# SamShue/EKF_SLAM

Hardware: AMD Instinct MI355X
Metric: EKF update-steps/sec at N landmarks; HBM GB/s on (I−KH)P vs roofline (higher is better)
Workload: dtype f64

## Files before the change

ekf_slam_amd/csrc/downdate.h:

```cpp
#pragma once

template <typename TS, int T, int kSlab>
__global__ __launch_bounds__(kBlock) void k_downdate(const TS *__restrict__ tiles, TS *__restrict__ dst,
                                                     const int2 *__restrict__ work, int64_t nwork,
                                                     const double *__restrict__ Kp, const double *__restrict__ Gp,
                                                     int64_t pair_stride, int pstart, int pcap, int npairs, TileMap tm) {
    using V2 = typename Vec2<TS>::type;
    constexpr int kPairsPerRow = T / 2;
    constexpr int kRowsPerPass = kBlock / kPairsPerRow;
    constexpr int kSlabsPerTile = T / kSlab;
    constexpr int kPasses = (kSlab + kRowsPerPass - 1) / kRowsPerPass;
    constexpr bool kExact = kRowsPerPass * kPasses == kSlab;
    static_assert(kPasses <= 8, "slab too tall for the register tile");
    const int tid = threadIdx.x;
    const int cp = tid % kPairsPerRow;
    const int r0 = tid / kPairsPerRow;
    const int64_t nitems = nwork * kSlabsPerTile;
    for (int64_t it0 = blockIdx.x; it0 < nitems; it0 += gridDim.x) {
        const int64_t it = tm.reverse ? nitems - 1 - it0 : it0;
        const int64_t w = it / kSlabsPerTile;
        const int slab = (int)(it - w * kSlabsPerTile);
        const int2 ij = work[w];
        const int64_t toff = tm.tile_offset(ij.x, ij.y) + (int64_t)slab * kSlab * T;
        const TS *__restrict__ tp = tiles + toff;
        TS *__restrict__ td = dst + toff;
        double2 v[kPasses];
#pragma unroll
        for (int p = 0; p < kPasses; ++p) {
            const int r = r0 + p * kRowsPerPass;
            if (kExact || r < kSlab) {
                const V2 t = *reinterpret_cast<const V2 *>(tp + r * T + 2 * cp);
                v[p] = make_double2((double)t.x, (double)t.y);
            }
        }
        const int64_t gcol = (int64_t)ij.y * T + 2 * cp;
        const int64_t krow = (int64_t)ij.x * T + slab * kSlab;
        for (int i = 0; i < npairs; ++i) {
            const int64_t so = (int64_t)ring_slot(pstart, i, pcap) * pair_stride;
            const double2 *__restrict__ g2 = reinterpret_cast<const double2 *>(Gp + so) + gcol;
            const double2 *__restrict__ k2 = reinterpret_cast<const double2 *>(Kp + so) + krow;
            const double2 ga = g2[0], gb = g2[1];
#pragma unroll
            for (int p = 0; p < kPasses; ++p) {
                const int r = r0 + p * kRowsPerPass;
                if (kExact || r < kSlab) {
                    const double2 k = k2[r];
                    v[p].x = rank2_apply(v[p].x, k, ga);
                    v[p].y = rank2_apply(v[p].y, k, gb);
                }
            }
        }
#pragma unroll
        for (int p = 0; p < kPasses; ++p) {
            const int r = r0 + p * kRowsPerPass;
            if (kExact || r < kSlab) {
                V2 o;
                o.x = (TS)v[p].x; o.y = (TS)v[p].y;
                *reinterpret_cast<V2 *>(td + r * T + 2 * cp) = o;
            }
        }
    }
}

template <typename TS> struct Lane16;
template <> struct Lane16<double> { using type = double2; static constexpr int kCols = 2; };
template <> struct Lane16<float>  { using type = float4;  static constexpr int kCols = 4; };
__device__ __forceinline__ void lane16_unpack(const double2 &t, double *v) { v[0] = t.x; v[1] = t.y; }
__device__ __forceinline__ void lane16_unpack(const float4 &t, double *v) { v[0] = t.x; v[1] = t.y; v[2] = t.z; v[3] = t.w; }
__device__ __forceinline__ void lane16_pack(const double *v, double2 &t) { t.x = v[0]; t.y = v[1]; }
__device__ __forceinline__ void lane16_pack(const double *v, float4 &t) {
    t.x = (float)v[0]; t.y = (float)v[1]; t.z = (float)v[2]; t.w = (float)v[3];
}
__device__ __forceinline__ double lane16_get(const double2 &t, int q) { return q == 0 ? t.x : t.y; }
__device__ __forceinline__ double lane16_get(const float4 &t, int q) { return (double)(q == 0 ? t.x : q == 1 ? t.y : q == 2 ? t.z : t.w); }

__device__ __attribute__((noinline)) void extract_next_row(double *__restrict__ send, int jm, int Ij, int tI, int tJ, int r, int c0, int ncols,
                                                           int T, int world, int rank, double v0, double v1, double v2, double v3) {
    const uint32_t wd = (uint32_t)world;
    const int k0 = (int)(((uint32_t)rank + wd - (uint32_t)Ij % wd) % wd);
    const bool rowtile = tI == Ij, coltile = tJ == Ij, diag = rowtile && coltile;
    for (int q = 0; q < ncols; ++q) {
        const int cc = c0 + q;
        const double val = q == 0 ? v0 : q == 1 ? v1 : q == 2 ? v2 : v3;
        if (rowtile && (r == jm || r == jm + 1)) {
            const int a = r - jm;
            if (!diag || cc <= jm) {
                const int64_t e = (int64_t)((tJ - k0) / world) * T + cc;
                send[2 * e + a] = val;
            }
            if (diag && a == 1 && (cc == jm || cc == jm + 1)) {
                const int64_t e = (int64_t)((Ij - k0) / world) * T + jm + 1;
                send[2 * e + (cc - jm)] = val;
            }
        }
        if (coltile && (cc == jm || cc == jm + 1) && (tI > Ij || r > jm + 1)) {
            const int64_t e = (int64_t)((tI - k0) / world) * T + r;
            send[2 * e + (cc - jm)] = val;
        }
    }
}

struct NoNextRow {};
template <bool kNext> struct NextRowParam { using type = NoNextRow; };
template <> struct NextRowParam<true> { using type = NextRow; };

template <typename TS, int T, int kSlab, bool kXcd, bool kNext = false>
__global__ __launch_bounds__(kBlock) void k_downdate_w(const TS *__restrict__ tiles, TS *__restrict__ dst,
                                                       const int2 *__restrict__ work, int64_t nwork,
                                                       const double *__restrict__ Kp, const double *__restrict__ Gp,
                                                       int64_t pair_stride, int pstart, int pcap, int npairs, TileMap tm,
                                                       typename NextRowParam<kNext>::type nx) {
    using VL = typename Lane16<TS>::type;
    constexpr int kCols = Lane16<TS>::kCols;
    constexpr int kLanesPerRow = T / kCols;
    constexpr int kRowsPerInstr = 64 / kLanesPerRow;
    constexpr int kRowsPerWave = kSlab / 4;
    constexpr int kPasses = kRowsPerWave / kRowsPerInstr;
    constexpr int kSlabsPerTile = T / kSlab;
    static_assert(kLanesPerRow == 64 || kLanesPerRow == 32, "tile edge / storage type combination not supported");
    static_assert(kPasses >= 1 && kPasses <= 8 && kPasses * kRowsPerInstr * 4 == kSlab, "bad slab");
    const int lane = threadIdx.x & 63;
    const int wave = __builtin_amdgcn_readfirstlane(threadIdx.x >> 6);
    const int sub = lane / kLanesPerRow;
    const int cl = lane % kLanesPerRow;
    const int64_t nitems = (kXcd ? 8 : 1) * nwork * kSlabsPerTile;
    const int64_t nv = nwork * kSlabsPerTile;
    for (int64_t it = blockIdx.x; it < nitems; it += gridDim.x) {
        const int64_t vf = kXcd ? (it >> 3) : it;
        const int64_t vi = tm.reverse ? nv - 1 - vf : vf;
        const int64_t w = vi / kSlabsPerTile;
        const int slab = (int)(vi - w * kSlabsPerTile);
        const int2 ij = work[kXcd ? (it & 7) * nwork + w : w];
        if (kXcd && ij.x < 0) continue;
        const int row0 = slab * kSlab + wave * kRowsPerWave;
        const int64_t toff = tm.tile_offset(ij.x, ij.y) + (int64_t)(row0 + sub) * T + kCols * cl;
        const TS *__restrict__ tp = tiles + toff;
        TS *__restrict__ td = dst + toff;
        double v[kPasses][kCols];
#pragma unroll
        for (int p = 0; p < kPasses; ++p) {
            const VL t = *reinterpret_cast<const VL *>(tp + (int64_t)p * kRowsPerInstr * T);
            lane16_unpack(t, v[p]);
        }
        const int64_t gcol = (int64_t)ij.y * T + kCols * cl;
        const int64_t krow = (int64_t)ij.x * T + row0;
        for (int i = 0; i < npairs; ++i) {
            const int64_t so = (int64_t)ring_slot(pstart, i, pcap) * pair_stride;
            const double2 *__restrict__ g2 = reinterpret_cast<const double2 *>(Gp + so) + gcol;
            const double2 *__restrict__ k2 = reinterpret_cast<const double2 *>(Kp + so) + krow;
            double2 g[kCols];
#pragma unroll
            for (int q = 0; q < kCols; ++q) g[q] = g2[q];
#pragma unroll
            for (int p = 0; p < kPasses; ++p) {
                double2 k = k2[p * kRowsPerInstr];
                if (kRowsPerInstr == 2) { const double2 k1 = k2[p * 2 + 1]; if (sub) k = k1; }
#pragma unroll
                for (int q = 0; q < kCols; ++q) v[p][q] = rank2_apply(v[p][q], k, g[q]);
            }
        }
        VL stored[kPasses];
#pragma unroll
        for (int p = 0; p < kPasses; ++p) {
            lane16_pack(v[p], stored[p]);
            *reinterpret_cast<VL *>(td + (int64_t)p * kRowsPerInstr * T) = stored[p];
        }
        if constexpr (kNext) {
            const int Ij = (int)(nx.j >> tm.shift);
            if (__builtin_expect(ij.x == Ij || ij.y == Ij, 0)) {
#pragma unroll
                for (int p = 0; p < kPasses; ++p) {
                    double vv[4] = { 0.0, 0.0, 0.0, 0.0 };
#pragma unroll
                    for (int q = 0; q < kCols; ++q) vv[q] = lane16_get(stored[p], q);
                    extract_next_row(nx.send, (int)(nx.j & (T - 1)), Ij, ij.x, ij.y, row0 + sub + p * kRowsPerInstr, kCols * cl, kCols, T,
                                     tm.world, tm.rank, vv[0], vv[1], vv[2], vv[3]);
                }
            }
        }
    }
}
```

ekf_slam_amd/csrc/flush64_mfma.h:

```cpp
#pragma once

typedef double d4_t __attribute__((ext_vector_type(4)));

template <typename TS, int T, int kChunk, int kCols = 128, int kWpe = (kChunk <= 4 ? 4 : 3), int kWaves = 4, int kAbl = 0>
__global__ __launch_bounds__(64 * kWaves) __attribute__((amdgpu_waves_per_eu(kWpe, kWpe)))
void k_flush_mfma(const TS *__restrict__ tiles, TS *__restrict__ dst, const int2 *__restrict__ work, int64_t nwork,
                  const double *__restrict__ Kp, const double *__restrict__ Gp, int64_t pair_stride, int pstart, int pcap,
                  int npairs, TileMap tm) {
    constexpr int kBlock = 64 * kWaves;
    constexpr int kRows = 16 * kWaves, kKPad = kRows + 16;
    constexpr int kE = 16 / (int)sizeof(TS);
    constexpr int kBP = kCols / (16 * kE);
    constexpr int kColParts = T / kCols, kSubsPerTile = (T / kRows) * kColParts;
    static_assert((kBP * kE == 8 || kBP * kE == 4) && T % kCols == 0 && T % kRows == 0, "a wavefront owns 16 rows x 128 (64) columns = 8 (4) MFMA blocks");
    static_assert(kChunk % 2 == 0 && (kChunk * kCols) % kBlock == 0 && (kChunk * kRows) % kBlock == 0, "bad chunk");
    __shared__ __attribute__((aligned(16))) double Gs[2 * kChunk][kCols];
    __shared__ double Ks[2 * kChunk][kKPad];
    const int tid = threadIdx.x;
    const int lane = tid & 63;
    const int wave = __builtin_amdgcn_readfirstlane(tid >> 6);
    const int lr = lane >> 4, lc = lane & 15;
    const int64_t nitems = 8 * nwork * kSubsPerTile;
    for (int64_t it = blockIdx.x; it < nitems; it += gridDim.x) {
        const int64_t vi = tm.reverse ? nwork * kSubsPerTile - 1 - (it >> 3) : (it >> 3);
        const int64_t w = vi / kSubsPerTile;
        const int sub = (int)(vi - w * kSubsPerTile);
        const int2 ij = work[(it & 7) * nwork + w];
        if (ij.x < 0) continue;
        const int slab = sub / kColParts, cpart = sub - slab * kColParts;
        const int row0 = slab * kRows + wave * 16;
        const int64_t toff = tm.tile_offset(ij.x, ij.y) + (int64_t)(row0 + lr) * T + cpart * kCols + kE * lc;
        const TS *__restrict__ tp = tiles + toff;
        TS *__restrict__ td = dst + toff;
        d4_t acc[kBP][kE];
#pragma unroll
        for (int bp = 0; bp < kBP; ++bp)
#pragma unroll
            for (int r = 0; r < 4; ++r)
#pragma unroll
                for (int e = 0; e < kE; ++e)
                    acc[bp][e][r] = (double)__builtin_nontemporal_load(tp + (int64_t)(4 * r) * T + 16 * kE * bp + e);
        const int64_t gcol0 = (int64_t)ij.y * T + cpart * kCols;
        const int64_t krow0 = (int64_t)ij.x * T + slab * kRows;
        constexpr int kPerG = kChunk * kCols / kBlock, kPerK = kChunk * kRows / kBlock;
        double2 tg[kPerG], tk[kPerK];
        auto fetch = [&](int c0, int cn) {
#pragma unroll
            for (int q = 0; q < kPerG; ++q) {
                const int e = tid + q * kBlock, col = e & (kCols - 1);
                const int i = (e / kCols) < cn ? (e / kCols) : cn - 1;
                tg[q] = reinterpret_cast<const double2 *>(Gp + (int64_t)ring_slot(pstart, c0 + i, pcap) * pair_stride)[gcol0 + col];
            }
#pragma unroll
            for (int q = 0; q < kPerK; ++q) {
                const int e = tid + q * kBlock, row = e & (kRows - 1);
                const int i = (e / kRows) < cn ? (e / kRows) : cn - 1;
                tk[q] = reinterpret_cast<const double2 *>(Kp + (int64_t)ring_slot(pstart, c0 + i, pcap) * pair_stride)[krow0 + row];
            }
        };
        if constexpr (kAbl < 2) fetch(0, npairs < kChunk ? npairs : kChunk);
        for (int c0 = 0; kAbl < 2 && c0 < npairs; c0 += kChunk) {
            const int cn = npairs - c0 < kChunk ? npairs - c0 : kChunk;
            __syncthreads();
#pragma unroll
            for (int q = 0; q < kPerG; ++q) {
                const int e = tid + q * kBlock, i = e / kCols, col = e & (kCols - 1);
                if (i < cn) { Gs[2 * i][col] = tg[q].x; Gs[2 * i + 1][col] = tg[q].y; }
                else if (i == cn) { Gs[2 * i][col] = 0.0; Gs[2 * i + 1][col] = 0.0; }
            }
#pragma unroll
            for (int q = 0; q < kPerK; ++q) {
                const int e = tid + q * kBlock, i = e / kRows, row = e & (kRows - 1);
                if (i < cn) { Ks[2 * i][row] = -tk[q].x; Ks[2 * i + 1][row] = -tk[q].y; }
                else if (i == cn) { Ks[2 * i][row] = -0.0; Ks[2 * i + 1][row] = -0.0; }
            }
            __syncthreads();
            if (c0 + kChunk < npairs) fetch(c0 + kChunk, npairs - c0 - kChunk < kChunk ? npairs - c0 - kChunk : kChunk);
            const int ksteps = kAbl ? 0 : (cn + 1) >> 1;
#pragma unroll 2
            for (int ks = 0; ks < ksteps; ++ks) {
                const double a = Ks[4 * ks + lr][wave * 16 + lc];
                double2 b[kBP][kE / 2];
// ... 27 lines not shown
```

ekf_slam_amd/csrc/host/handle.h:

```cpp
#pragma once
#include "../../../include/ekfslam.h"
#include <hip/hip_runtime.h>
#include <dlfcn.h>
#include <cstdio>
#include <cstdlib>
#include <algorithm>
#include <cmath>
#include <cstring>
#include <new>
#include <string>
#include <vector>

#include "../device_math.h"
#include "../flush32_pipe.h"
#include "../kernels.h"
#include "../layout.h"

struct KernelTimer {
    bool enabled = false;
    std::vector<hipEvent_t> ev;
    size_t used = 0;
};

struct ekf_handle {
    ekf_config cfg;
    int64_t N = 0;
    int64_t cap = 0;
    int32_t T = 64;
    int32_t storage = 0;
    int32_t cur = 0;
    DevState st;
    hipStream_t own_stream = nullptr, stream = nullptr;
    double *h_small = nullptr;
    double *d_digest = nullptr;
    bool have_pp = false;
    PredictArgs pp;
    std::vector<double> s_host;
    mutable std::vector<std::pair<double, int64_t>> s_sorted, s_tail;
    mutable bool s_sorted_ok = false;
    static constexpr size_t kSortedTail = 2048;
    hipEvent_t throttle_ev[2] = { nullptr, nullptr };
    bool throttle_set[2] = { false, false };
    int throttle_k = 0, since_mark = 0;
    int32_t batch = 1;
    int32_t npend = 0;
    int32_t pstart = 0;
    bool async_flush = false;
    void *tilebuf[2] = { nullptr, nullptr };
    int32_t base = 0;
    int32_t nfrozen = 0;
    bool inflight = false;
    int64_t inflight_N = 0;
    bool appended_inflight = false;
    const int64_t *inflight_dn = nullptr;
    int flush_cus = 0;
    hipStream_t flush_stream = nullptr;
    hipEvent_t ev_pairs = nullptr, ev_flushed = nullptr, ev_rows = nullptr;
    PassAux aux = { nullptr, 0, nullptr, 0, 0, nullptr, nullptr };
    int grid_cap = 0;
    char dd_kernel[64] = "";
    int32_t dd_pairs = 0;
    struct WorkSet {
        int2 *work = nullptr;
        int64_t nwork = 0;
        int2 *xcd = nullptr;
        int64_t xcd_len = 0;
        int4 *segs = nullptr;
        int64_t nsegs = 0, cols = 0;
        int64_t rows = -1;
    };
    WorkSet ws[2];
    int32_t ws_cur = 0;
    int32_t ws_pass = -1;
    bool ws_unordered = false;
    int64_t work_cap = 0, segs_cap = 0;
    char *wl_stage = nullptr;
    size_t wl_stage_bytes = 0;
    hipEvent_t ev_wl = nullptr;
    bool wl_busy = false;
    AssocDecision *d_partial = nullptr, *d_decision = nullptr, *h_decision = nullptr;
    AssocDecision *h_decision_dev = nullptr;
    int *d_ticket = nullptr;
    double *d_pos_cost = nullptr, *d_sig_cost = nullptr;
    int32_t assoc_seq = 0;
    static constexpr int kSpecRing = 64;
    AssocHostPartial *h_parts = nullptr, *h_parts_dev = nullptr;
    int64_t parts_stride = 0;
    bool assoc_poll = true;
    struct Spec { int32_t seq, is_new, nblk; int64_t idx, idx_N; };
    std::vector<Spec> spec;
    static constexpr int kLoopRing = 256;
    AssocHostPartial *d_lparts = nullptr;
    int64_t lparts_stride = 0;
    int32_t loop_set = 0;
    AssocHostPartial *h_lrec = nullptr, *h_lrec_dev = nullptr;
    struct LoopSpec { int32_t seq, is_new; int64_t idx; };
    std::vector<LoopSpec> lspec;
    uint64_t lrec_head = 0, lrec_tail = 0;
    static constexpr int kNRing = 1024;
    int64_t *d_nring = nullptr;
    uint64_t nrow = 0;
    static constexpr int kTabSets = 64, kTabCap = 512;
    double *h_loctab = nullptr, *h_loctab_dev = nullptr;
    int32_t *d_abort = nullptr;
    int32_t scan_id = 0;
    int64_t lookup_fail_hits = -1;
    uint64_t tab_until[kTabSets] = {};
    bool tab_used[kTabSets] = {};
    int tab_next = 0;
    bool sharded = false;
    double *own_send = nullptr, *own_recv = nullptr, *send = nullptr, *recv = nullptr;
    int64_t slab_cap = 0;
    int64_t xchg_cap = 0;
    int64_t slab = 0;
    bool pending = false;
    bool assoc_costs = false;
    int pending_kind = 0;
// ... 162 lines not shown
```

ekf_slam_amd/csrc/host/passes.h:

```cpp
#pragma once
namespace {
int32_t refresh_work(ekf_handle *h) {
    const int64_t nt = ekf_tiles_for(2 * n_hi(h), h->T);
    if (nt == h->ws[h->ws_cur].rows) return EKF_OK;
    const int32_t to = h->ws_pass == h->ws_cur ? h->ws_cur ^ 1 : h->ws_cur;
    ekf_handle::WorkSet &ws = h->ws[to];
    const size_t b_work = (size_t)h->work_cap * sizeof(int2), b_xcd = 8 * b_work, b_segs = (size_t)h->segs_cap * sizeof(int4);
    if (!h->wl_stage) h->wl_stage_bytes = b_work + b_xcd + b_segs;
    int32_t rc = stage_alloc(h, &h->wl_stage, h->wl_stage_bytes, &h->ev_wl);
    if (!rc) rc = stage_wait(h, h->ev_wl, h->wl_busy);
    if (rc) return rc;
    int2 *w = reinterpret_cast<int2 *>(h->wl_stage);
    int2 *flat = reinterpret_cast<int2 *>(h->wl_stage + b_work);
    int4 *segs = reinterpret_cast<int4 *>(h->wl_stage + b_work + b_xcd);
    size_t nw = 0;
    REQUIRE(h, h->st.tm.slots_for_rows(nt) <= h->work_cap, EKF_ERR_STATE, "work list overflow");
    for (int64_t I = 0; I < nt; ++I)
        for (int64_t J = 0; J <= I; ++J)
            if (h->st.tm.mine(I, J)) w[nw++] = make_int2((int)I, (int)J);
    if (nw) HIPCHK(h, hipMemcpyAsync(ws.work, w, nw * sizeof(int2), hipMemcpyHostToDevice, h->stream));
    ws.nwork = (int64_t)nw;
    ws.rows = nt;

    static const int S = std::max(1, ekf_tune_int("EKF_SUPERTILE", 8));
    struct Super { int64_t si, sj; std::vector<int2> tiles; };
    std::vector<Super> supers;
    const int64_t ns = (nt + S - 1) / S;
    for (int64_t si = 0; si < ns; ++si)
        for (int64_t sj = 0; sj <= si; ++sj) {
            Super sp; sp.si = si; sp.sj = sj;
            for (int64_t I = si * S; I < nt && I < (si + 1) * S; ++I)
                for (int64_t J = sj * S; J <= I && J < (sj + 1) * S; ++J)
                    if (h->st.tm.mine(I, J)) sp.tiles.push_back(make_int2((int)I, (int)J));
            if (!sp.tiles.empty()) supers.push_back(std::move(sp));
        }
    static const int order = ekf_tune_int("EKF_XCD_ORDER", 1);
    std::vector<int2> stream[8];
    if (order == 0) {
        std::stable_sort(supers.begin(), supers.end(), [](const Super &a, const Super &b) { return a.tiles.size() > b.tiles.size(); });
        for (const Super &sp : supers) {
            int best = 0;
            for (int x = 1; x < 8; ++x) if (stream[x].size() < stream[best].size()) best = x;
            stream[best].insert(stream[best].end(), sp.tiles.begin(), sp.tiles.end());
        }
    } else {
        std::vector<int2> flat_order;
        flat_order.reserve(nw);
        for (const Super &sp : supers) flat_order.insert(flat_order.end(), sp.tiles.begin(), sp.tiles.end());
        const size_t tot = flat_order.size();
        for (int x = 0; x < 8; ++x)
            stream[x].assign(flat_order.begin() + (tot * x) / 8, flat_order.begin() + (tot * (x + 1)) / 8);
    }
    size_t len = 0;
    for (int x = 0; x < 8; ++x) len = std::max(len, stream[x].size());
    REQUIRE(h, (int64_t)(8 * len) <= 8 * h->work_cap, EKF_ERR_STATE, "XCD work list overflow");
    std::fill(flat, flat + 8 * len, make_int2(-1, -1));
    for (int x = 0; x < 8; ++x) std::copy(stream[x].begin(), stream[x].end(), flat + x * len);
    if (len) HIPCHK(h, hipMemcpyAsync(ws.xcd, flat, 8 * len * sizeof(int2), hipMemcpyHostToDevice, h->stream));
    ws.xcd_len = (int64_t)len;
    if (ws.segs) {
        std::vector<int4> sg;
        const int64_t nsegs = ekf_pipe32::build_strip_segments(h->st.tm, nt, sg);
        REQUIRE(h, (int64_t)sg.size() <= h->segs_cap, EKF_ERR_STATE, "strip work list overflow");
        if (!sg.empty()) {
            std::copy(sg.begin(), sg.end(), segs);
            HIPCHK(h, hipMemcpyAsync(ws.segs, segs, sg.size() * sizeof(int4), hipMemcpyHostToDevice, h->stream));
        }
        ws.nsegs = nsegs;
        ws.cols = nt * h->T;
    }
    TRY(stage_uploaded(h, h->ev_wl, h->wl_busy));
    h->ws_cur = to;
    h->ws_unordered = true;
    return EKF_OK;
}

const PassAux *pass_aux(const ekf_handle *h, const ekf_handle::WorkSet &ws, PassAux &out) {
    if (!ws.segs) return nullptr;
    out = h->aux;
    out.segs = ws.segs; out.nsegs = ws.nsegs; out.cols = ws.cols;
    return &out;
}

PassJob pass_job(const ekf_handle *h, const ekf_handle::WorkSet &ws, void *dst, PassAux &ax) {
    PassJob job = {};
    job.dst = dst;
    job.work = ws.work; job.nwork = ws.nwork; job.work_xcd = ws.xcd; job.xcd_len = ws.xcd_len;
    job.pstart = h->pstart; job.npairs = h->npend;
    job.grid_cap = h->grid_cap; job.arith = h->cfg.pass_arith;
    job.aux = pass_aux(h, ws, ax);
    return job;
}

int32_t create_worklists(ekf_handle *h) {
    for (auto &ws : h->ws) {
        if (h->cfg.pass_arith != EKF_ARITH_F64) HIPCHK(h, dalloc(h, &ws.segs, (size_t)h->segs_cap));
        HIPCHK(h, dalloc(h, &ws.work, (size_t)h->work_cap));
        HIPCHK(h, dalloc(h, &ws.xcd, (size_t)h->work_cap * 8));
    }
    return EKF_OK;
}

int32_t retire_inflight(ekf_handle *h) {
    if (!h->inflight) return EKF_OK;
    if (h->appended_inflight) {
        if (!h->ev_rows) HIPCHK(h, new_event(h, &h->ev_rows));
        HIPCHK(h, hipEventRecord(h->ev_rows, h->stream));
        HIPCHK(h, hipStreamWaitEvent(h->flush_stream, h->ev_rows, 0));
        if (decided_mode(h)) {
            const int64_t *hi = unsettled(h) > 0 ? h->d_nring + h->nrow % ekf_handle::kNRing : nullptr;
            HIPCHK(h, launch_copy_rows_dev(h->st.tm, h->tilebuf[h->base], h->tilebuf[h->base ^ 1], 2 * h->inflight_N, 2 * n_hi(h), h->inflight_dn,
                                           hi, h->storage, h->flush_stream));
        } else
            HIPCHK(h, launch_copy_rows(h->st.tm, h->tilebuf[h->base], h->tilebuf[h->base ^ 1], 2 * h->inflight_N, 2 * h->N, h->storage, h->flush_stream));
        HIPCHK(h, hipEventRecord(h->ev_flushed, h->flush_stream));
        h->appended_inflight = false;
    }
    HIPCHK(h, hipStreamWaitEvent(h->stream, h->ev_flushed, 0));
    h->ws_pass = -1;
    h->base ^= 1;
    h->st.tiles = h->tilebuf[h->base];
    h->pstart = (h->pstart + h->nfrozen) % h->st.pcap;
    h->npend -= h->nfrozen;
    h->nfrozen = 0;
    h->inflight = false;
    tiles_changed(h);
    return EKF_OK;
}

void next_pass_direction(ekf_handle *h) {
    const int force = h->cfg.pass_direction == 1 ? 0 : h->cfg.pass_direction == 2 ? 1 : -1;
    constexpr int64_t kCacheBytes = 256ll << 20;
    const int64_t nt = ekf_tiles_for(2 * n_hi(h), h->T);
    const int64_t store = nt * (nt + 1) / 2 / std::max(1, h->cfg.world) * (int64_t)h->T * h->T * (h->storage == EKF_STORE_F64 ? 8 : 4);
    const bool alternate = force >= 0 ? force != 0 : store > kCacheBytes;
    h->st.tm.reverse = alternate ? (h->st.tm.reverse ^ 1) : 0;
}

int32_t flush_pending(ekf_handle *h, bool batch_done = false) {
    TRY(retire_inflight(h));
    if (h->npend == 0) return EKF_OK;
    TRY(refresh_work(h));
    next_pass_direction(h);
    bool extracted = false;
    const int64_t hint = h->hint_idx;
    bool pn = false, pn_side = false;
    if (batch_done && !h->pn_idx.empty()) {
        if (h->sharded && !h->pending && h->pn_N == h->N && (h->comm || h->xhook)) {
            const int32_t m = (int32_t)h->pn_idx.size();
            const int64_t slab = slab_for(h, n_mm(h));
            TIMED(h, EKF_KERNEL_ROWPANEL, launch_rowpanel_next(h->st, h->pn_idx.data(), m, n_mm(h), h->pstart, h->npend, h->send, slab, h->storage,
                  h->stream));
            tiles_changed(h);
            h->pf_idx = h->pn_idx; h->pf_m = m; h->pf_slab = slab; h->pf_N = h->N;
            h->x_count = (int64_t)m * slab;
            static const int pn_side_stream = ekf_tune_int("EKF_PN_SIDE_STREAM", 0);
            if (h->comm) {
                pn_side = pn_side_stream != 0;
                if (pn_side && !h->xchg_stream) {
                    HIPCHK(h, hipStreamCreateWithFlags(&h->xchg_stream, hipStreamNonBlocking));
                    HIPCHK(h, new_event(h, &h->ev_pn_ready));
                    HIPCHK(h, new_event(h, &h->ev_pn_done));
                }
                if (pn_side) {
                    HIPCHK(h, hipEventRecord(h->ev_pn_ready, h->stream));
                    HIPCHK(h, hipStreamWaitEvent(h->xchg_stream, h->ev_pn_ready, 0));
                }
                const hipStream_t xs = pn_side ? h->xchg_stream : h->stream;
                const int r = g_rccl.AllGather(h->send, h->recv, (size_t)h->x_count,  8, h->comm, xs);
                if (r != 0) return fail(h, EKF_ERR_COMM, g_rccl.GetErrorString(r));
                HIPCHK(h, store_panels(h, xs));
                if (pn_side) HIPCHK(h, hipEventRecord(h->ev_pn_done, h->xchg_stream));
            } else {
                TRY(exchange_bracket(h, 2));
                HIPCHK(h, store_panels(h, h->stream));
            }
            pn = true;
        }
        drop_announced(h);
    }
    {
        NextRow nx = { -1, nullptr };
        if (h->sharded && h->npend == 1 && !h->pending && hint >= 0 && hint < h->N) {
            nx.j = 2 * hint;
            nx.send = corr_send(h, slab_for(h, n_mm(h)));
        }
        TimedLaunch tl(h, EKF_KERNEL_DOWNDATE);
        const ekf_handle::WorkSet &ws = h->ws[h->ws_cur];
        PassAux ax;
        PassJob job = pass_job(h, ws, h->st.tiles, ax);
        job.nx = nx.j >= 0 ? &nx : nullptr;
        HIPCHK(h, launch_downdate(h->st, job, h->storage, h->stream, h->dd_kernel, &extracted));
        h->dd_pairs = h->npend;
    }
    h->npend = 0;
    h->pstart = 0;
    h->pf_valid = pn;
    if (pn_side) HIPCHK(h, hipStreamWaitEvent(h->stream, h->ev_pn_done, 0));
    h->nx_valid = extracted && !pn;
    if (extracted) { h->nx_idx = hint; h->nx_N = h->N; }
    return EKF_OK;
}

int32_t batch_complete(ekf_handle *h) {
    if (!h->async_flush) return flush_pending(h,  true);
    HIPCHK(h, hipEventRecord(h->ev_pairs, h->stream));
    h->ws_unordered = false;
    TRY(retire_inflight(h));
    TRY(refresh_work(h));
    HIPCHK(h, hipStreamWaitEvent(h->flush_stream, h->ev_pairs, 0));
    if (h->ws_unordered) HIPCHK(h, hipStreamWaitEvent(h->flush_stream, h->ev_wl, 0));
    {
        TimedLaunch tl(h, EKF_KERNEL_DOWNDATE, h->flush_stream);
        next_pass_direction(h);
        const ekf_handle::WorkSet &ws = h->ws[h->ws_cur];
        PassAux ax;
        HIPCHK(h, launch_downdate(h->st, pass_job(h, ws, h->tilebuf[h->base ^ 1], ax), h->storage, h->flush_stream, h->dd_kernel));
        h->dd_pairs = h->npend;
    }
    HIPCHK(h, hipEventRecord(h->ev_flushed, h->flush_stream));
    h->nfrozen = h->npend;
    h->inflight = true;
    h->ws_pass = h->ws_cur;
    h->inflight_N = h->N;
    h->inflight_dn = unsettled(h) > 0 ? h->d_nring + h->nrow % ekf_handle::kNRing : nullptr;
    h->appended_inflight = false;
    return EKF_OK;
}

int32_t create_passes(ekf_handle *h, const hipDeviceProp_t &prop) {
    const ekf_config &cfg = h->cfg;
    const int32_t T = h->T;
    const int64_t ldm = h->st.ldm, slots = h->work_cap, nt_cap = ldm / T;
    char *tiles = nullptr;
    HIPCHK(h, dalloc(h, &tiles, (size_t)slots * T * T * elt_size(h)));
    h->st.tiles = tiles;
    h->tilebuf[0] = tiles;
    h->async_flush = cfg.async_flush != 0;
    if (h->async_flush) {
        char *tiles2 = nullptr;
        HIPCHK(h, dalloc(h, &tiles2, (size_t)slots * T * T * elt_size(h)));
        h->tilebuf[1] = tiles2;
        int reserve = ekf_tune_int("EKF_ASYNC_RESERVE_CUS", cfg.pass_arith == EKF_ARITH_SPLIT3 ? 64 : 32);
        const int ncu = prop.multiProcessorCount;
// ... 49 lines not shown
```

ekf_slam_amd/csrc/kernels.h:

```cpp
#pragma once
#include <hip/hip_runtime.h>
#include <stdint.h>

#include "device_math.h"
#include "assign_math.h"
#include "kernel_args.h"
#include "layout.h"

#ifdef EKF_TUNING
#include <stdlib.h>
inline int ekf_tune_int(const char *name, int dflt) { const char *v = getenv(name); return v ? atoi(v) : dflt; }
#else
constexpr int ekf_tune_int(const char *, int dflt) { return dflt; }
#endif

hipError_t launch_predict(const DevState &st, const PredictArgs &a, int storage, hipStream_t s);

hipError_t launch_predict_model(const DevState &st, const PredictModelArgs &a, hipStream_t s);

hipError_t launch_append(const DevState &st, const AppendArgs &a, int storage, hipStream_t s, const DevLoopArgs *dl = nullptr,
                         const PredictArgs *fused_predict = nullptr);

hipError_t launch_append_model(const DevState &st, const AppendModelArgs &a, int storage, hipStream_t s);

// ... 46 lines not shown
struct alignas(16) AssocHostPartial {
    double  min_ll;
    int32_t index;
    int32_t tag;
};
#if defined(__HIPCC__)
__host__ __device__
#endif
inline uint32_t assoc_part_mix(uint32_t ll_lo, uint32_t ll_hi, uint32_t index) {
    uint32_t m = ll_lo * 0x9E3779B1u ^ (ll_hi + 0x7F4A7C15u) * 0x85EBCA6Bu ^ (index + 0x165667B1u) * 0xC2B2AE35u;
    m ^= m >> 15; m *= 0x2C1B3C6Du; m ^= m >> 13;
    return m;
}

constexpr int kAssocBlock = 256;

hipError_t launch_associate(const DevState &st, const AssocArgs &a, double *pos_cost, double *sig_cost,
                            AssocDecision *partial, int *ticket, AssocDecision *decision, AssocHostPartial *host_partials, int seq,
                            double *cand, int storage, hipStream_t s, const PredictArgs *fused_predict = nullptr);
hipError_t launch_associate_devn(const DevState &st, const AssocArgs &a, AssocHostPartial *host_partials, int seq, int storage,
                                 hipStream_t s, const PredictArgs *fused_predict);
hipError_t launch_assoc_merge(const DevState &st, const double *recv, int world, int64_t count, int64_t N, bool want_costs,
                              double *pos_cost, AssocDecision *decision, AssocDecision *host_decision, int seq, hipStream_t s);

hipError_t launch_assoc_model(const DevState &st, const AssocModelArgs &a, ekfm::Match2 *partials, ekfm::Match2 *out, double *d2_all,
                              hipStream_t s);

hipError_t launch_assign_model(const DevState &st, const AssocModelArgs &a, ekfm::Match2 *partials, ekfm::CandList *lists, ekfm::CandList *sel,
                               AssignResult *res, hipStream_t s);
hipError_t launch_assign_lists(const DevState &st, const AssocModelArgs &a, ekfm::Match2 *partials, ekfm::CandList *lists, ekfm::CandList *sel,
                               AssignResult *res, hipStream_t s);

struct NextRow { int64_t j; double *send; };
struct PassAux {
    const int4 *segs;
    int64_t nsegs;
    float *dump;
    int grid;
    int64_t cols;
    uint16_t *Kb3, *Gb3;
};
size_t pass_split_plane_elems(int64_t ldm);
struct PassJob {
    void *dst;
    const int2 *work;
    int64_t nwork;
    const int2 *work_xcd;
    int64_t xcd_len;
    int pstart, npairs;
    int grid_cap;
    int arith;
    const PassAux *aux;
    const NextRow *nx;
};
hipError_t launch_downdate(const DevState &st, const PassJob &job, int storage, hipStream_t s, char *kname, bool *extracted = nullptr);
hipError_t launch_copy_rows(const TileMap &tm, const void *src, void *dst, int64_t r0, int64_t r1, int storage, hipStream_t s);
hipError_t launch_copy_rows_dev(const TileMap &tm, const void *src, void *dst, int64_t r0, int64_t r1, const int64_t *n_lo,
                                const int64_t *n_hi, int storage, hipStream_t s);

hipError_t launch_compact_tiles(const TileMap &tm, const void *src, void *dst, const int2 *work, int64_t ntiles, const int32_t *src_of,
                                int storage, hipStream_t s);
hipError_t launch_compact_state(const DevState &st, int cur, const int32_t *src_of, int64_t N_old, double *s_out, hipStream_t s);
hipError_t launch_constrain_probe(const DevState &st, int cur, int64_t ai, int64_t aj, double *out, int storage, hipStream_t s);
hipError_t launch_gather_constrain(const DevState &st, const ConstrainArgs &a, int storage, hipStream_t s);
hipError_t launch_gather_constrain_chain(const DevState &st, const ConstrainArgs &a, double *rec, int storage, hipStream_t s);
hipError_t launch_merge_pass(const DevState &st, void *dst, const int2 *work, int64_t ntiles, const int32_t *src_of, int npairs,
                             int storage, hipStream_t s, char *kname);
hipError_t launch_nearest(const DevState &st, int cur, int64_t N, const double R[4], NearestEntry *out, int storage, hipStream_t s);

hipError_t launch_gather_linear(const DevState &st, const LinearArgs &a, double *rec, int64_t *cnt, int storage, hipStream_t s);
hipError_t launch_linear_probe(const DevState &st, const LinearArgs &a, double *rec, int storage, hipStream_t s);

hipError_t launch_gather_model(const DevState &st, const ModelArgs &a, double *rec, int64_t *cnt, int storage, hipStream_t s);
hipError_t launch_model_probe(const DevState &st, const ModelArgs &a, double *rec, int storage, hipStream_t s);
hipError_t launch_gather_model_assigned(const DevState &st, const AssignedModelArgs &a, const AssignedRecord *slot, double *rec, int64_t *cnt,
                                        int storage, hipStream_t s);
hipError_t launch_gather_model_iter(const DevState &st, const IterModelArgs &a, double *rec, int64_t *cnt, double *itrec, int storage, hipStream_t s);
hipError_t launch_model_iter_probe(const DevState &st, const IterModelArgs &a, double *rec, double *itrec, int storage, hipStream_t s);

hipError_t launch_joint_innovation(const DevState &st, const JointArgs &a, const int64_t *hyp, int nh, JointRecord *out, double *d2_prefix,
                                   double *nu, double *S, int storage, hipStream_t s);

hipError_t launch_joint_search_prepare(const DevState &st, const JointArgs &a, const ekfm::CandList *sel, const int64_t *match,
                                       JointSearchStore *store, JointSearchOut *out, hipStream_t s);
hipError_t launch_joint_search_level(const DevState &st, const JointSearchArgs &a, const JointSearchLevelArgs &la, const ekfm::CandList *sel,
                                     JointSearchStore *store, JointSearchOut *out, int which, int storage, hipStream_t s);

hipError_t launch_joint_factor(const DevState &st, const JointArgs &a, const int64_t *hyp, JointBlock *blk, JointRecord *out, double *nu, double *S,
                               int storage, hipStream_t s);
hipError_t launch_joint_factor_iter(const DevState &st, const JointArgs &a, const JointIterArgs &ia, const int64_t *hyp, JointBlock *blk,
                                    JointRecord *out, double *itrec, double *nu, double *S, int storage, hipStream_t s);
hipError_t launch_gather_joint(const DevState &st, const JointUpdateArgs &a, const JointBlock *blk, int storage, hipStream_t s);

hipError_t launch_unpack_dense(const DevState &st, int cur, int64_t n_mm, double *dense, int storage, hipStream_t s);
hipError_t launch_pack_dense(const DevState &st, int cur, int64_t n_mm, const double *dense, int storage, hipStream_t s);
hipError_t launch_get_block(const DevState &st, int cur, int64_t r0, int64_t c0, int64_t nr, int64_t nc,
                            double *out, int storage, hipStream_t s);
hipError_t launch_get_diag_blocks(const DevState &st, int cur, int64_t N, double *out, int storage, hipStream_t s);
hipError_t launch_lowrank(const DevState &st, int cur, int64_t n_mm, const int2 *work, int64_t nwork, const double *d,
                          const double *U, int64_t k, int storage, hipStream_t s);
constexpr int kDigestGrid = 2048;
constexpr int kDigestDoubles = 4 + 3 * kDigestGrid;
hipError_t launch_digest(const DevState &st, int cur, int64_t n_mm, const int2 *work, int64_t nwork, double *out,
                         int storage, hipStream_t s);
```

ekf_slam_amd/csrc/kernels.hip:

```cpp
#include "kernels.h"

#include <algorithm>
#include <atomic>
#include <cstdio>
#include <type_traits>

#include "device_math.h"
#include "flush32_mfma.h"
#include "flush32_pipe.h"
#include "flush32_split.h"
#include "flush64_mfma.h"

namespace {

#include "tile_access.h"
#include "lane_ops.h"
#include "predict.h"
#include "predict_model.h"
#include "assoc_winners.h"
#include "append.h"
#include "append_model.h"
#include "join_map.h"
#include "extract_map.h"
#include "solve_small.h"
#include "rowpanel.h"
#include "pair_column.h"
#include "gather.h"
#include "downdate.h"
#include "associate.h"
#include "state_io.h"
#include "compact.h"
#include "transform_map.h"
#include "constrain.h"
#include "linear_obs.h"
#include "model_obs.h"
#include "model_assigned.h"
#include "model_iter.h"
#include "associate_model.h"
#include "assign_model.h"
#include "joint.h"
#include "joint_search.h"
#include "joint_update.h"
#include "joint_iter.h"
#include "merge_pass.h"
#include "nearest.h"
#include "factor_map.h"
#include "sample_map.h"

}

#include "launch/dispatch.h"
#include "launch/steps.h"
#include "launch/pass_select.h"
#include "launch/passes.h"
#include "launch/edits.h"
#include "launch/state_io.h"
// ... 1 lines not shown
```

ekf_slam_amd/csrc/launch/passes.h:

```cpp
#pragma once

size_t pass_split_plane_elems(int64_t ldm) { return ekf_pipe32::split_plane_elems(ldm); }

namespace {
hipError_t allow_dynamic_lds(const void *fn, size_t bytes, std::atomic<uint64_t> &done) {
    int dev = 0;
    hipError_t e = hipGetDevice(&dev);
    if (e != hipSuccess) return e;
    const uint64_t bit = 1ull << (dev & 63);
    if (done.load(std::memory_order_acquire) & bit) return hipSuccess;
    e = hipFuncSetAttribute(fn, hipFuncAttributeMaxDynamicSharedMemorySize, (int)bytes);
    if (e == hipSuccess) done.fetch_or(bit, std::memory_order_release);
    return e;
}

template <typename TS_, int kT, int kSlab> struct PassShape { using TS = TS_; static constexpr int T = kT, slab = kSlab; };
template <typename... S> struct PassShapes {};
using ValuShapes = PassShapes<
    PassShape<double, 16, 16>, PassShape<double, 32, 16>, PassShape<double, 32, 32>,
    PassShape<double, 64, 8>, PassShape<double, 64, 16>, PassShape<double, 64, 32>, PassShape<double, 64, 64>,
    PassShape<double, 128, 4>, PassShape<double, 128, 8>, PassShape<double, 128, 16>, PassShape<double, 128, 32>,
    PassShape<float, 16, 16>, PassShape<float, 32, 32>, PassShape<float, 64, 64>, PassShape<float, 128, 8>, PassShape<float, 128, 64>,
    PassShape<float, 256, 4>, PassShape<float, 256, 8>, PassShape<float, 256, 16>, PassShape<float, 256, 32>>;

template <typename F, typename... S> bool with_shape(PassShapes<S...>, const ekf_pass::PassInstance &p, F &&f) {
    return (((int)sizeof(typename S::TS) == p.elt && S::T == p.T && S::slab == p.slab ? (f(S{}), true) : false) || ...);
}
}

hipError_t launch_downdate(const DevState &st, const PassJob &job, int storage, hipStream_t s, char *kname, bool *extracted) {
    using namespace ekf_pass;
    if (extracted) *extracted = false;
    if (job.nwork <= 0 || job.npairs <= 0) return hipSuccess;
    static const int slab1 = ekf_tune_int("EKF_DOWNDATE_SLAB", 0);
    static const int slabm = ekf_tune_int("EKF_DOWNDATE_SLAB_BATCH", 0);
    static const PassKnobs knobs = { ekf_tune_int("EKF_FLUSH_MFMA", 1) != 0, ekf_tune_int("EKF_FLUSH_MFMA_SWITCH", 30), ekf_tune_int("EKF_FLUSH_HALF_MAX", 12),
                                     ekf_tune_int("EKF_PASS_STRIP", 1) != 0, ekf_tune_int("EKF_FLUSH_XCD", 1) != 0 };
    const PassAux *aux = job.aux;
    const int T = st.tm.T, pstart = job.pstart, npairs = job.npairs;
    PassQuery q = { storage == 0 ? 8 : 4, T, npairs, job.arith,  job.work_xcd && job.xcd_len > 0,
                     aux && aux->segs && aux->nsegs > 0,  aux && aux->Kb3 && aux->Gb3,  job.nx && job.nx->j >= 0,
                     npairs > 1 ? slabm : slab1 };
    PassInstance p = select_pass(q, knobs);
    static std::atomic<uint64_t> split_ok{0}, strip_ok{0};
    if (p.family == kSplit3 && allow_dynamic_lds((const void *)ekf_pipe32::k_flush_split3<2>, ekf_pipe32::lds_bytes_split(), split_ok) != hipSuccess) {
        q.planes = false;
        p = select_pass(q, knobs);
    }
    if (p.family == kStrip32 && allow_dynamic_lds((const void *)ekf_pipe32::k_flush_strip32<8>, ekf_pipe32::lds_bytes_strip<8>(), strip_ok) != hipSuccess) {
        q.strip_list = false;
        p = select_pass(q, knobs);
    }

    auto flush = [&](auto kernel, auto ts, auto *Kp, auto *Gp, int rows, int cols) {
        using TS = decltype(ts);
        hipLaunchKernelGGL(kernel, dim3(clamp_grid(8 * job.xcd_len * (T / rows) * (T / cols), job.grid_cap)), dim3(kBlock), 0, s,
                           (const TS *)st.tiles, (TS *)job.dst, job.work_xcd, job.xcd_len, Kp, Gp, st.pair_stride, pstart, st.pcap, npairs, st.tm);
    };
    switch (p.family) {
        case kInvalid: return hipErrorInvalidValue;
        case kSplit3:
            hipLaunchKernelGGL(ekf_pipe32::k_split_pairs, dim3((unsigned)(aux->cols / 256), ekf_pipe32::kKB, 2), dim3(256), 0, s, (const float *)st.Kp32,
                               (const float *)st.Gp32, aux->Kb3, aux->Gb3, st.pair_stride, st.ldm, aux->cols, pstart, st.pcap, npairs);
            hipLaunchKernelGGL((ekf_pipe32::k_flush_split3<2>), dim3((unsigned)aux->grid), dim3(512), ekf_pipe32::lds_bytes_split(), s,
                               (const float *)st.tiles, (float *)job.dst, aux->segs, aux->nsegs, (const uint16_t *)aux->Kb3, (const uint16_t *)aux->Gb3, st.ldm,
                               st.tm, aux->dump);
            break;
        case kStrip32:
            hipLaunchKernelGGL((ekf_pipe32::k_flush_strip32<8>), dim3((unsigned)aux->grid), dim3(512), ekf_pipe32::lds_bytes_strip<8>(), s,
                               (const float *)st.tiles, (float *)job.dst, aux->segs, aux->nsegs, (const float *)st.Kp32, (const float *)st.Gp32, st.pair_stride,
                               st.ldm, pstart, st.pcap, npairs, st.tm, aux->dump, (unsigned long long *)nullptr);
            break;
        case kMfma32:
            if (p.early) flush(k_flush_mfma32<256, 4, 2, 3, true>, float{}, st.Kp32, st.Gp32, 128, 128);
            else flush(k_flush_mfma32<256, 4, 2, 3>, float{}, st.Kp32, st.Gp32, 128, 128);
            break;
        case kMfma64:
            if (p.elt == 4) {
                if (p.chunk == 4) flush(k_flush_mfma<float, 256, 4>, float{}, st.Kp, st.Gp, 64, 128);
                else flush(k_flush_mfma<float, 256, 8>, float{}, st.Kp, st.Gp, 64, 128);
            } else if (p.cols == 64) flush(k_flush_mfma<double, 128, 4, 64, 5>, double{}, st.Kp, st.Gp, 64, 64);
            else if (p.chunk == 4) flush(k_flush_mfma<double, 128, 4>, double{}, st.Kp, st.Gp, 64, 128);
            else flush(k_flush_mfma<double, 128, 8>, double{}, st.Kp, st.Gp, 64, 128);
            break;
        case kDowndateW:
        case kDowndate: {
            const bool built = with_shape(ValuShapes{}, p, [&](auto shape) {
                using TS = typename decltype(shape)::TS;
                constexpr int kT = decltype(shape)::T, kSlab = decltype(shape)::slab, kLanes = kT / Lane16<TS>::kCols;
                const TS *src = (const TS *)st.tiles;
                TS *dst = (TS *)job.dst;
                const dim3 grid(clamp_grid(job.nwork * (kT / kSlab), job.grid_cap)), grid_xcd(clamp_grid(8 * job.xcd_len * (kT / kSlab), job.grid_cap));
                if constexpr (kLanes != 64 && kLanes != 32) {
                    hipLaunchKernelGGL((k_downdate<TS, kT, kSlab>), grid, dim3(kBlock), 0, s, src, dst, job.work, job.nwork, st.Kp, st.Gp,
                                       st.pair_stride, pstart, st.pcap, npairs, st.tm);
                } else {
                    auto per_row = [&](auto kernel, dim3 g, const int2 *list, int64_t n, auto next) {
                        hipLaunchKernelGGL(kernel, g, dim3(kBlock), 0, s, src, dst, list, n, st.Kp, st.Gp, st.pair_stride, pstart, st.pcap, npairs, st.tm, next);
                    };
                    if (p.xcd) per_row(k_downdate_w<TS, kT, kSlab, true>, grid_xcd, job.work_xcd, job.xcd_len, NoNextRow{});
                    else if (p.rowpanel) per_row(k_downdate_w<TS, kT, kSlab, false, true>, grid, job.work, job.nwork, *job.nx);
                    else per_row(k_downdate_w<TS, kT, kSlab, false>, grid, job.work, job.nwork, NoNextRow{});
                }
            });
            if (!built) return hipErrorInvalidValue;
            if (extracted) *extracted = p.rowpanel;
            break;
        }
    }
    if (kname) snprintf(kname, 64, "%s", p.name);
    return hipGetLastError();
}

namespace {
template <typename Launch>
hipError_t copy_tile_rows(const TileMap &tm, int64_t r0, int64_t r1, int storage, Launch &&launch) {
    if (r1 <= r0) return hipSuccess;
    const int T = tm.T;
    if (T > kBlock * (storage == 0 ? 2 : 4)) return hipErrorInvalidValue;
    hipError_t e = hipSuccess;
    for (int64_t I = r0 >> tm.shift; I <= (r1 - 1) >> tm.shift; ++I) {
        const int64_t lo = std::max<int64_t>(r0, I * T) - I * T, hi = std::min<int64_t>(r1, (I + 1) * T) - I * T;
        const int64_t slot0 = tm.row_base(I), nslots = tm.row_base(I + 1) - slot0;
        if (nslots <= 0 || hi <= lo) continue;
        const int lanes = T / (storage == 0 ? 2 : 4), per_wg = kBlock / lanes > 0 ? kBlock / lanes : 1;
        const hipError_t ei = launch(dim3((unsigned)cdiv(nslots * (hi - lo), per_wg)), slot0, nslots, (int)lo, (int)(hi - lo), I);
        if (ei != hipSuccess) e = ei;
    }
    return e;
}
}

hipError_t launch_copy_rows(const TileMap &tm, const void *src, void *dst, int64_t r0, int64_t r1, int storage, hipStream_t s) {
    return copy_tile_rows(tm, r0, r1, storage, [&](dim3 grid, int64_t slot0, int64_t nslots, int lo, int n, int64_t) {
        return with_storage(storage, [&](auto ts) {
            using TS = decltype(ts);
            hipLaunchKernelGGL(k_copy_tile_rows<TS>, grid, dim3(kBlock), 0, s, (const TS *)src, (TS *)dst, slot0, nslots, lo, n, tm.T);
        });
    });
}

hipError_t launch_copy_rows_dev(const TileMap &tm, const void *src, void *dst, int64_t r0, int64_t r1, const int64_t *n_lo,
                                const int64_t *n_hi, int storage, hipStream_t s) {
    return copy_tile_rows(tm, r0, r1, storage, [&](dim3 grid, int64_t slot0, int64_t nslots, int lo, int n, int64_t I) {
        return with_storage(storage, [&](auto ts) {
            using TS = decltype(ts);
            hipLaunchKernelGGL(k_copy_tile_rows_dev<TS>, grid, dim3(kBlock), 0, s, (const TS *)src, (TS *)dst, slot0, nslots, lo, n, tm.T,
                               I * tm.T, r0, r1, n_lo, n_hi);
        });
    });
}
```

Baseline: 1932.

## Skip dead rows beyond live state in downdate and flush kernels

Passes the live row count (twice the active landmark count) into the downdate and MFMA flush kernels so slabs entirely past the live covariance rows are skipped. For the per-row downdate kernel, the last tile row's work items are compacted with a smaller per-tile slab count (tail_shift), so fewer grid items are scheduled for the partially filled final tile row. Index math switches to 32-bit for the non-XCD path. This adds host-side bookkeeping (head of the work list) and a size guard, and it risks mis-indexing if the head or tail layout does not match the work list.

```diff
diff --git a/ekf_slam_amd/csrc/downdate.h b/ekf_slam_amd/csrc/downdate.h
--- a/ekf_slam_amd/csrc/downdate.h
+++ b/ekf_slam_amd/csrc/downdate.h
@@ -4,7 +4,7 @@
 __global__ __launch_bounds__(kBlock) void k_downdate(const TS *__restrict__ tiles, TS *__restrict__ dst,
                                                      const int2 *__restrict__ work, int64_t nwork,
                                                      const double *__restrict__ Kp, const double *__restrict__ Gp,
-                                                     int64_t pair_stride, int pstart, int pcap, int npairs, TileMap tm) {
+                                                     int64_t pair_stride, int pstart, int pcap, int npairs, TileMap tm, int live) {
     using V2 = typename Vec2<TS>::type;
     constexpr int kPairsPerRow = T / 2;
     constexpr int kRowsPerPass = kBlock / kPairsPerRow;
@@ -21,6 +21,7 @@
         const int64_t w = it / kSlabsPerTile;
         const int slab = (int)(it - w * kSlabsPerTile);
         const int2 ij = work[w];
+        if (ij.x * T + slab * kSlab >= live) continue;
         const int64_t toff = tm.tile_offset(ij.x, ij.y) + (int64_t)slab * kSlab * T;
         const TS *__restrict__ tp = tiles + toff;
         TS *__restrict__ td = dst + toff;
@@ -109,7 +110,7 @@
                                                        const int2 *__restrict__ work, int64_t nwork,
                                                        const double *__restrict__ Kp, const double *__restrict__ Gp,
                                                        int64_t pair_stride, int pstart, int pcap, int npairs, TileMap tm,
-                                                       typename NextRowParam<kNext>::type nx) {
+                                                       typename NextRowParam<kNext>::type nx, int live, int head, int tail_shift) {
     using VL = typename Lane16<TS>::type;
     constexpr int kCols = Lane16<TS>::kCols;
     constexpr int kLanesPerRow = T / kCols;
@@ -119,19 +120,35 @@
     constexpr int kSlabsPerTile = T / kSlab;
     static_assert(kLanesPerRow == 64 || kLanesPerRow == 32, "tile edge / storage type combination not supported");
     static_assert(kPasses >= 1 && kPasses <= 8 && kPasses * kRowsPerInstr * 4 == kSlab, "bad slab");
+    static_assert((kSlabsPerTile & (kSlabsPerTile - 1)) == 0, "slabs per tile: a power of two");
     const int lane = threadIdx.x & 63;
     const int wave = __builtin_amdgcn_readfirstlane(threadIdx.x >> 6);
     const int sub = lane / kLanesPerRow;
     const int cl = lane % kLanesPerRow;
-    const int64_t nitems = (kXcd ? 8 : 1) * nwork * kSlabsPerTile;
-    const int64_t nv = nwork * kSlabsPerTile;
-    for (int64_t it = blockIdx.x; it < nitems; it += gridDim.x) {
-        const int64_t vf = kXcd ? (it >> 3) : it;
-        const int64_t vi = tm.reverse ? nv - 1 - vf : vf;
-        const int64_t w = vi / kSlabsPerTile;
-        const int slab = (int)(vi - w * kSlabsPerTile);
-        const int2 ij = work[kXcd ? (it & 7) * nwork + w : w];
+    __builtin_assume(npairs > 0);
+    using Index = typename std::conditional<kXcd, int64_t, uint32_t>::type;
+    const Index nv = kXcd ? (Index)(nwork * kSlabsPerTile) : (Index)(head + (((int)nwork - head / kSlabsPerTile) << tail_shift));
+    const Index nitems = (kXcd ? 8 : 1) * nv;
+    for (Index it = blockIdx.x; it < nitems; it += gridDim.x) {
+        const Index vf = kXcd ? (it >> 3) : it;
+        const Index vi = tm.reverse ? nv - 1 - vf : vf;
+        int64_t w;
+        int slab;
+        if (kXcd) {
+            w = vi / kSlabsPerTile;
+            slab = (int)(vi - w * kSlabsPerTile);
+        } else {
+            const int u = (int)vi, t = u - head;
+            const bool tail = u >= head;
+            const int sh = tail ? tail_shift : __builtin_ctz(kSlabsPerTile), un = tail ? t : u;
+            w = (tail ? head / kSlabsPerTile : 0) + (un >> sh);
+            slab = un & ((1 << sh) - 1);
+        }
+        const uint64_t e = *reinterpret_cast<const uint64_t *>(work + (kXcd ? (it & 7) * nwork + w : w));
+        const int2 ij = make_int2((int)(uint32_t)e, (int)(uint32_t)(e >> 32));
         if (kXcd && ij.x < 0) continue;
+        const int first = ij.x * T + slab * kSlab;
+        if (first >= live) continue;
         const int row0 = slab * kSlab + wave * kRowsPerWave;
         const int64_t toff = tm.tile_offset(ij.x, ij.y) + (int64_t)(row0 + sub) * T + kCols * cl;
         const TS *__restrict__ tp = tiles + toff;
@@ -143,7 +160,7 @@
             lane16_unpack(t, v[p]);
         }
         const int64_t gcol = (int64_t)ij.y * T + kCols * cl;
-        const int64_t krow = (int64_t)ij.x * T + row0;
+        const int64_t krow = first + wave * kRowsPerWave;
         for (int i = 0; i < npairs; ++i) {
             const int64_t so = (int64_t)ring_slot(pstart, i, pcap) * pair_stride;
             const double2 *__restrict__ g2 = reinterpret_cast<const double2 *>(Gp + so) + gcol;
diff --git a/ekf_slam_amd/csrc/flush64_mfma.h b/ekf_slam_amd/csrc/flush64_mfma.h
--- a/ekf_slam_amd/csrc/flush64_mfma.h
+++ b/ekf_slam_amd/csrc/flush64_mfma.h
@@ -6,7 +6,7 @@
 __global__ __launch_bounds__(64 * kWaves) __attribute__((amdgpu_waves_per_eu(kWpe, kWpe)))
 void k_flush_mfma(const TS *__restrict__ tiles, TS *__restrict__ dst, const int2 *__restrict__ work, int64_t nwork,
                   const double *__restrict__ Kp, const double *__restrict__ Gp, int64_t pair_stride, int pstart, int pcap,
-                  int npairs, TileMap tm) {
+                  int npairs, TileMap tm, int live) {
     constexpr int kBlock = 64 * kWaves;
     constexpr int kRows = 16 * kWaves, kKPad = kRows + 16;
     constexpr int kE = 16 / (int)sizeof(TS);
@@ -28,6 +28,7 @@
         const int2 ij = work[(it & 7) * nwork + w];
         if (ij.x < 0) continue;
         const int slab = sub / kColParts, cpart = sub - slab * kColParts;
+        if (ij.x * T + slab * kRows >= live) continue;
         const int row0 = slab * kRows + wave * 16;
         const int64_t toff = tm.tile_offset(ij.x, ij.y) + (int64_t)(row0 + lr) * T + cpart * kCols + kE * lc;
         const TS *__restrict__ tp = tiles + toff;
diff --git a/ekf_slam_amd/csrc/host/handle.h b/ekf_slam_amd/csrc/host/handle.h
--- a/ekf_slam_amd/csrc/host/handle.h
+++ b/ekf_slam_amd/csrc/host/handle.h
@@ -63,6 +63,7 @@
     struct WorkSet {
         int2 *work = nullptr;
         int64_t nwork = 0;
+        int64_t nwork_head = 0;
         int2 *xcd = nullptr;
         int64_t xcd_len = 0;
         int4 *segs = nullptr;
diff --git a/ekf_slam_amd/csrc/host/passes.h b/ekf_slam_amd/csrc/host/passes.h
--- a/ekf_slam_amd/csrc/host/passes.h
+++ b/ekf_slam_amd/csrc/host/passes.h
@@ -15,11 +15,15 @@
     int4 *segs = reinterpret_cast<int4 *>(h->wl_stage + b_work + b_xcd);
     size_t nw = 0;
     REQUIRE(h, h->st.tm.slots_for_rows(nt) <= h->work_cap, EKF_ERR_STATE, "work list overflow");
-    for (int64_t I = 0; I < nt; ++I)
+    size_t nw_head = 0;
+    for (int64_t I = 0; I < nt; ++I) {
+        if (I == nt - 1) nw_head = nw;
         for (int64_t J = 0; J <= I; ++J)
             if (h->st.tm.mine(I, J)) w[nw++] = make_int2((int)I, (int)J);
+    }
     if (nw) HIPCHK(h, hipMemcpyAsync(ws.work, w, nw * sizeof(int2), hipMemcpyHostToDevice, h->stream));
     ws.nwork = (int64_t)nw;
+    ws.nwork_head = (int64_t)nw_head;
     ws.rows = nt;
 
     static const int S = std::max(1, ekf_tune_int("EKF_SUPERTILE", 8));
@@ -85,7 +89,7 @@
 PassJob pass_job(const ekf_handle *h, const ekf_handle::WorkSet &ws, void *dst, PassAux &ax) {
     PassJob job = {};
     job.dst = dst;
-    job.work = ws.work; job.nwork = ws.nwork; job.work_xcd = ws.xcd; job.xcd_len = ws.xcd_len;
+    job.work = ws.work; job.nwork = ws.nwork; job.nwork_head = ws.nwork; job.work_xcd = ws.xcd; job.xcd_len = ws.xcd_len;
     job.pstart = h->pstart; job.npairs = h->npend;
     job.grid_cap = h->grid_cap; job.arith = h->cfg.pass_arith;
     job.aux = pass_aux(h, ws, ax);
@@ -190,6 +194,8 @@
         PassAux ax;
         PassJob job = pass_job(h, ws, h->st.tiles, ax);
         job.nx = nx.j >= 0 ? &nx : nullptr;
+        job.live_rows = 2 * n_hi(h);
+        if (ekf_tiles_for(job.live_rows, h->T) == ws.rows) job.nwork_head = ws.nwork_head;
         HIPCHK(h, launch_downdate(h->st, job, h->storage, h->stream, h->dd_kernel, &extracted));
         h->dd_pairs = h->npend;
     }
diff --git a/ekf_slam_amd/csrc/kernels.h b/ekf_slam_amd/csrc/kernels.h
--- a/ekf_slam_amd/csrc/kernels.h
+++ b/ekf_slam_amd/csrc/kernels.h
@@ -122,6 +122,8 @@
     int arith;
     const PassAux *aux;
     const NextRow *nx;
+    int64_t live_rows;
+    int64_t nwork_head;
 };
 hipError_t launch_downdate(const DevState &st, const PassJob &job, int storage, hipStream_t s, char *kname, bool *extracted = nullptr);
 hipError_t launch_copy_rows(const TileMap &tm, const void *src, void *dst, int64_t r0, int64_t r1, int storage, hipStream_t s);
diff --git a/ekf_slam_amd/csrc/kernels.hip b/ekf_slam_amd/csrc/kernels.hip
--- a/ekf_slam_amd/csrc/kernels.hip
+++ b/ekf_slam_amd/csrc/kernels.hip
@@ -2,6 +2,7 @@
 
 #include <algorithm>
 #include <atomic>
+#include <climits>
 #include <cstdio>
 #include <type_traits>
 
diff --git a/ekf_slam_amd/csrc/launch/passes.h b/ekf_slam_amd/csrc/launch/passes.h
--- a/ekf_slam_amd/csrc/launch/passes.h
+++ b/ekf_slam_amd/csrc/launch/passes.h
@@ -38,6 +38,7 @@
                                      ekf_tune_int("EKF_PASS_STRIP", 1) != 0, ekf_tune_int("EKF_FLUSH_XCD", 1) != 0 };
     const PassAux *aux = job.aux;
     const int T = st.tm.T, pstart = job.pstart, npairs = job.npairs;
+    const int live = job.live_rows > 0 && job.live_rows < INT_MAX ? (int)job.live_rows : INT_MAX;
     PassQuery q = { storage == 0 ? 8 : 4, T, npairs, job.arith,  job.work_xcd && job.xcd_len > 0,
                      aux && aux->segs && aux->nsegs > 0,  aux && aux->Kb3 && aux->Gb3,  job.nx && job.nx->j >= 0,
                      npairs > 1 ? slabm : slab1 };
@@ -52,10 +53,10 @@
         p = select_pass(q, knobs);
     }
 
-    auto flush = [&](auto kernel, auto ts, auto *Kp, auto *Gp, int rows, int cols) {
+    auto flush = [&](auto kernel, auto ts, auto *Kp, auto *Gp, int rows, int cols, auto... more) {
         using TS = decltype(ts);
         hipLaunchKernelGGL(kernel, dim3(clamp_grid(8 * job.xcd_len * (T / rows) * (T / cols), job.grid_cap)), dim3(kBlock), 0, s,
-                           (const TS *)st.tiles, (TS *)job.dst, job.work_xcd, job.xcd_len, Kp, Gp, st.pair_stride, pstart, st.pcap, npairs, st.tm);
+                           (const TS *)st.tiles, (TS *)job.dst, job.work_xcd, job.xcd_len, Kp, Gp, st.pair_stride, pstart, st.pcap, npairs, st.tm, more...);
     };
     switch (p.family) {
         case kInvalid: return hipErrorInvalidValue;
@@ -77,14 +78,15 @@
             break;
         case kMfma64:
             if (p.elt == 4) {
-                if (p.chunk == 4) flush(k_flush_mfma<float, 256, 4>, float{}, st.Kp, st.Gp, 64, 128);
-                else flush(k_flush_mfma<float, 256, 8>, float{}, st.Kp, st.Gp, 64, 128);
-            } else if (p.cols == 64) flush(k_flush_mfma<double, 128, 4, 64, 5>, double{}, st.Kp, st.Gp, 64, 64);
-            else if (p.chunk == 4) flush(k_flush_mfma<double, 128, 4>, double{}, st.Kp, st.Gp, 64, 128);
-            else flush(k_flush_mfma<double, 128, 8>, double{}, st.Kp, st.Gp, 64, 128);
+                if (p.chunk == 4) flush(k_flush_mfma<float, 256, 4>, float{}, st.Kp, st.Gp, 64, 128, live);
+                else flush(k_flush_mfma<float, 256, 8>, float{}, st.Kp, st.Gp, 64, 128, live);
+            } else if (p.cols == 64) flush(k_flush_mfma<double, 128, 4, 64, 5>, double{}, st.Kp, st.Gp, 64, 64, live);
+            else if (p.chunk == 4) flush(k_flush_mfma<double, 128, 4>, double{}, st.Kp, st.Gp, 64, 128, live);
+            else flush(k_flush_mfma<double, 128, 8>, double{}, st.Kp, st.Gp, 64, 128, live);
             break;
         case kDowndateW:
         case kDowndate: {
+            bool oversize = false;
             const bool built = with_shape(ValuShapes{}, p, [&](auto shape) {
                 using TS = typename decltype(shape)::TS;
                 constexpr int kT = decltype(shape)::T, kSlab = decltype(shape)::slab, kLanes = kT / Lane16<TS>::kCols;
@@ -93,17 +95,29 @@
                 const dim3 grid(clamp_grid(job.nwork * (kT / kSlab), job.grid_cap)), grid_xcd(clamp_grid(8 * job.xcd_len * (kT / kSlab), job.grid_cap));
                 if constexpr (kLanes != 64 && kLanes != 32) {
                     hipLaunchKernelGGL((k_downdate<TS, kT, kSlab>), grid, dim3(kBlock), 0, s, src, dst, job.work, job.nwork, st.Kp, st.Gp,
-                                       st.pair_stride, pstart, st.pcap, npairs, st.tm);
+                                       st.pair_stride, pstart, st.pcap, npairs, st.tm, live);
                 } else {
+                    constexpr int kSlabs = kT / kSlab;
+                    int64_t head = job.nwork * kSlabs, items = head;
+                    int tail_shift = 0;
+                    if (live != INT_MAX && job.nwork_head >= 0 && job.nwork_head < job.nwork) {
+                        const int in_last = live - (live - 1) / kT * kT, slabs = (in_last + kSlab - 1) / kSlab;
+                        while ((1 << tail_shift) < slabs) ++tail_shift;
+                        head = job.nwork_head * kSlabs;
+                        items = head + ((job.nwork - job.nwork_head) << tail_shift);
+                    }
+                    if (!p.xcd && items > INT_MAX) { oversize = true; return; }
+                    const dim3 grid_list(clamp_grid(items, job.grid_cap));
                     auto per_row = [&](auto kernel, dim3 g, const int2 *list, int64_t n, auto next) {
-                        hipLaunchKernelGGL(kernel, g, dim3(kBlock), 0, s, src, dst, list, n, st.Kp, st.Gp, st.pair_stride, pstart, st.pcap, npairs, st.tm, next);
+                        hipLaunchKernelGGL(kernel, g, dim3(kBlock), 0, s, src, dst, list, n, st.Kp, st.Gp, st.pair_stride, pstart, st.pcap, npairs, st.tm, next, live,
+                                           (int)head, tail_shift);
                     };
                     if (p.xcd) per_row(k_downdate_w<TS, kT, kSlab, true>, grid_xcd, job.work_xcd, job.xcd_len, NoNextRow{});
-                    else if (p.rowpanel) per_row(k_downdate_w<TS, kT, kSlab, false, true>, grid, job.work, job.nwork, *job.nx);
-                    else per_row(k_downdate_w<TS, kT, kSlab, false>, grid, job.work, job.nwork, NoNextRow{});
+                    else if (p.rowpanel) per_row(k_downdate_w<TS, kT, kSlab, false, true>, grid_list, job.work, job.nwork, *job.nx);
+                    else per_row(k_downdate_w<TS, kT, kSlab, false>, grid_list, job.work, job.nwork, NoNextRow{});
                 }
             });
-            if (!built) return hipErrorInvalidValue;
+            if (!built || oversize) return hipErrorInvalidValue;
             if (extracted) *extracted = p.rowpanel;
             break;
         }
```

Measured after the change: 1955, median of 6. 1.2% higher.
